# Atten4Vis/LW-DETR

Hardware: AMD Instinct MI355X
Metric: images/sec (higher is better)
Workload: dtype fp16; 1 GPU; LW-DETR-small inference forward + PostProcess, 640x640, batch 32/GPU, fp16, random-init weights (synthetic COCO-shaped input); global_batch=32, per_gpu_batch=32, parallelism=dp1, collective=none, launch_chains=2

## Files before the change

lw-detr_amd/csrc/mlp.hip:

```cpp
#include "common.h"
#include "vit_block_few384.h"
#include <atomic>
#include <cstdlib>
#include <type_traits>

#ifndef MLP_WAVES_PER_SIMD
#define MLP_WAVES_PER_SIMD 2
#endif

#define TSTAMP(i) do {} while (0)

namespace {

#ifndef MLP_NW
#define MLP_NW 8
#endif
#ifndef MLP_TT384
#define MLP_TT384 1
#endif
constexpr int NW = MLP_NW, NTHR = NW * 64;

__device__ __forceinline__ void dma16(const void* sbase, unsigned voff, const void* lds_wave_base) {
    const unsigned m0v = __builtin_amdgcn_readfirstlane(
        (unsigned)(uintptr_t)(__attribute__((address_space(3))) const void*)lds_wave_base);
    asm volatile("s_mov_b32 m0, %0\n\ts_nop 0\n\tglobal_load_lds_dwordx4 %1, %2" :: "s"(m0v), "v"(voff), "s"(sbase) : "memory");
}
__device__ __forceinline__ const void* uniform_ptr(const void* p) {
    const uintptr_t v = (uintptr_t)p;
    const unsigned lo = __builtin_amdgcn_readfirstlane((unsigned)v), hi = __builtin_amdgcn_readfirstlane((unsigned)(v >> 32));
    return (const void*)(((uintptr_t)hi << 32) | lo);
}
__device__ __forceinline__ void dma_sync() {
    asm volatile("s_waitcnt vmcnt(0)" ::: "memory");
    __syncthreads();
}

struct MlpParams {
    void* x; long ldx;
    const void* w1; const float* b1;
    const void* w2p; const float* b2;
    const float* gamma2;
    void* out2; long ld2;
    float* stats_out;
    long M; float eps, eps_next;
    int ntiles;
    const void* att; long ldatt; const void* wp; const float* bp; const float* gamma1;
    const void* wqkv; const float* bqkv; void* q; void* k; void* vt; float qscale; int heads, hd, Tp;
    float* partial; int chunks_per_split;
    int wfrag;
};

constexpr int MP_COUNT = 44;
std::atomic<long> g_mlp_path[MP_COUNT];
const char* const kMlpPathNames[MP_COUNT] = {
    "mlp_f16_c192_proj0_qkv0", "mlp_f16_c192_proj1_qkv0", "mlp_f16_c192_proj1_qkv1", "mlp_f16_c384_proj0_qkv0", "mlp_f16_c384_proj1_qkv0",
    "mlp_f16_c384_proj1_qkv1", "mlp_bf16_c192_proj0_qkv0", "mlp_bf16_c192_proj1_qkv0", "mlp_bf16_c192_proj1_qkv1", "mlp_bf16_c384_proj0_qkv0",
    "mlp_bf16_c384_proj1_qkv0", "mlp_bf16_c384_proj1_qkv1", "mlp_f32_c192_proj0_qkv0", "mlp_f32_c192_proj1_qkv0", "mlp_f32_c192_proj1_qkv1",
    "mlp_f32_c384_proj0_qkv0", "mlp_f32_c384_proj1_qkv0", "mlp_f32_c384_proj1_qkv1", "mlp_small_f16_tt1_qkv0_frag0", "mlp_small_f16_tt1_qkv0_frag1",
    "mlp_small_f16_tt1_qkv1_frag0", "mlp_small_f16_tt1_qkv1_frag1", "mlp_small_f16_tt2_qkv0_frag0", "mlp_small_f16_tt2_qkv0_frag1", "mlp_small_f16_tt2_qkv1_frag0",
    "mlp_small_f16_tt2_qkv1_frag1", "mlp_small_bf16_tt1_qkv0_frag0", "mlp_small_bf16_tt1_qkv0_frag1", "mlp_small_bf16_tt1_qkv1_frag0",
    "mlp_small_bf16_tt1_qkv1_frag1", "mlp_small_bf16_tt2_qkv0_frag0", "mlp_small_bf16_tt2_qkv0_frag1", "mlp_small_bf16_tt2_qkv1_frag0",
    "mlp_small_bf16_tt2_qkv1_frag1", "mlp_small_f32_tt1_qkv0_frag1", "mlp_small_f32_tt1_qkv1_frag1", "vit_few384_f16_qkv0", "vit_few384_f16_qkv1",
    "vit_few384_bf16_qkv0", "vit_few384_bf16_qkv1", "ffn_f16_c256", "ffn_f16_c384", "ffn_bf16_c256", "ffn_bf16_c384"};
template <typename T> constexpr int mp_dt() { return std::is_same<T, f16>::value ? 0 : (std::is_same<T, bf16>::value ? 1 : 2); }
template <typename T, int C, bool PROJ, bool QKV> constexpr int mp_mlp() {
    static_assert((C == 192 || C == 384) && (PROJ || !QKV), "a form the record has no name for");
    return (mp_dt<T>() * 2 + (C == 384 ? 1 : 0)) * 3 + (PROJ ? (QKV ? 2 : 1) : 0);
}
template <typename T, bool QKV, int TT, bool FRAG> constexpr int mp_small() {
    static_assert(TT == 1 || TT == 2, "");
    static_assert(mp_dt<T>() < 2 || (TT == 1 && FRAG), "the f32 few-token kernel is built with TT = 1 on fragment-major weights only");
    return mp_dt<T>() == 2 ? 34 + (QKV ? 1 : 0) : 18 + ((mp_dt<T>() * 2 + (TT - 1)) * 2 + (QKV ? 1 : 0)) * 2 + (FRAG ? 1 : 0);
}
inline int mp_few384(int dtype, bool qkv) { return 36 + (dtype == DT_F16 ? 0 : 2) + (qkv ? 1 : 0); }
template <typename T, int C> constexpr int mp_ffn() {
    static_assert(mp_dt<T>() < 2 && (C == 256 || C == 384), "");
    return 40 + mp_dt<T>() * 2 + (C == 384 ? 1 : 0);
}
inline int mlp_path_done(int path, int rc) {
    if (rc == LWDETR_OK && path >= 0 && path < MP_COUNT) g_mlp_path[path].fetch_add(1, std::memory_order_relaxed);
    return rc;
}

template <typename T, int C, int TT, bool PROJ, bool QKV, bool FFN = false>
__global__ __launch_bounds__(NTHR, MLP_WAVES_PER_SIMD) void mlp_kernel(const MlpParams p) {
    static_assert(!FFN || (!PROJ && !QKV), "FFN mode has no projection / chained QKV");
    typedef typename Vec<T>::v8 V8;
    typedef typename Vec<T>::v4 V4;
    constexpr int KC = C / 32;
    constexpr int NT = C / 16;
    constexpr int HID = 4 * C, NCH = HID / 32;
    constexpr int EPC = 16 / (int)sizeof(T);
    constexpr int W1_LD = C + 2 * EPC;
// ... 104 lines not shown
        V8 af[TT][KC];
#pragma unroll
        for (int t = 0; t < TT; ++t) {
            long m = m_wave + t * 16 + l15; m = m < p.M ? m : p.M - 1;
            const T* ar = ATT + m * p.ldatt + g * 8;
#pragma unroll
            for (int kc = 0; kc < KC; ++kc) af[t][kc] = *(const V8*)(ar + kc * 32);
        }
        dma_sync();
#pragma unroll
        for (int pc = 0; pc < KC; ++pc) {
            const int buf = pc & 1;
            if (pc + 1 < KC) stage_rows32(WP + (long)(pc + 1) * 32 * C, buf ^ 1);
            else stage_w(0, buf ^ 1);
            const T* wps = smem + buf * TILE_STRIDE;
            f32x4 accp[2][TT];
#pragma unroll
            for (int h = 0; h < 2; ++h)
#pragma unroll
                for (int t = 0; t < TT; ++t) accp[h][t] = f32x4{0.f, 0.f, 0.f, 0.f};
#pragma unroll
            for (int kc = 0; kc < KC; ++kc)
#pragma unroll
                for (int h = 0; h < 2; ++h) {
                    const V8 a = *(const V8*)(wps + (h * 16 + l15) * W1_LD + kc * 32 + g * 8);
#pragma unroll
                    for (int t = 0; t < TT; ++t) accp[h][t] = Mma<T>::k32(a, af[t][kc], accp[h][t]);
                }
#pragma unroll
            for (int h = 0; h < 2; ++h) {
                const int c0 = pc * 32 + h * 16 + g * 4;
                const f32x4 bb = *(const f32x4*)(bps + c0), gg = *(const f32x4*)(bps + C + c0);
#pragma unroll
                for (int t = 0; t < TT; ++t) {
                    const long m = m_wave + t * 16 + l15;
                    const long mr = m < p.M ? m : p.M - 1;
                    V4 x1;
                    if (X1LDS) {
                        T* xs = x1s + (t * 16 + l15) * X1_LD + c0;
                        x1 = cvt4<T>(up4<T>(*(const V4*)xs) + gg * (accp[h][t] + bb));
                        if (wave < X1_TILES) *(V4*)xs = x1;
                    } else {
                        x1 = cvt4<T>(up4<T>(*(const V4*)(X + mr * p.ldx + c0)) + gg * (accp[h][t] + bb));
                        if (m < p.M) *(V4*)(X + m * p.ldx + c0) = x1;
                    }
#pragma unroll
                    for (int e = 0; e < 4; ++e) xf[t][pc][h * 4 + e] = x1[e];
                }
            }
            dma_sync();
        }
    }
    TSTAMP(1);
#pragma unroll
    for (int t = 0; t < (FFN ? 0 : TT); ++t) {
        float s = 0.f;
#pragma unroll
        for (int kc = 0; kc < KC; ++kc)
#pragma unroll
            for (int e = 0; e < 8; ++e) s += to_f32<T>(xf[t][kc][e]);
        s += __shfl_xor(s, 16); s += __shfl_xor(s, 32);
        const float mean = s * (1.f / C);
        float v = 0.f;
#pragma unroll
        for (int kc = 0; kc < KC; ++kc)
#pragma unroll
            for (int e = 0; e < 8; ++e) { const float dl = to_f32<T>(xf[t][kc][e]) - mean; v += dl * dl; }
        v += __shfl_xor(v, 16); v += __shfl_xor(v, 32);
        const float rstd = 1.f / sqrtf(v * (1.f / C) + p.eps);
#pragma unroll
        for (int kc = 0; kc < KC; ++kc)
#pragma unroll
            for (int e = 0; e < 8; ++e) xf[t][kc][e] = from_f32<T>((to_f32<T>(xf[t][kc][e]) - mean) * rstd);
    }

    f32x4 acc2[NT][TT];
#pragma unroll
    for (int n = 0; n < NT; ++n)
#pragma unroll
        for (int t = 0; t < TT; ++t) acc2[n][t] = f32x4{0.f, 0.f, 0.f, 0.f};

    if (!PROJ) dma_sync();
    TSTAMP(2);
    for (int hc = hc0; hc < hc1; ++hc) {
        const int buf = (hc - hc0) & 1;
        if (hc + 1 < hc1) stage_w(hc + 1, buf ^ 1);
        const T* w1s = smem + buf * TILE_STRIDE;
        const T* w2s = w1s + W1_TILE_PAD;
        const f32x4 bia0 = *(const f32x4*)(b1s + (hc - hc0) * 32 + g * 4), bia1 = *(const f32x4*)(b1s + (hc - hc0) * 32 + 16 + g * 4);
        constexpr int RD = 3, NF1 = 2 * KC, NF = NF1 + NT;
        auto frag = [&](int i) -> V8 {
            if (i < NF1) return *(const V8*)(w1s + ((i & 1) * 16 + l15) * W1_LD + (i >> 1) * 32 + g * 8);
            return *(const V8*)(w2s + ((i - NF1) * 16 + l15) * W2_LD + g * 8);
        };
        V8 fr[RD];
#pragma unroll
        for (int i = 0; i < RD; ++i) fr[i] = frag(i);
        f32x4 acc1[2][TT];
#pragma unroll
        for (int t = 0; t < TT; ++t) { acc1[0][t] = bia0; acc1[1][t] = bia1; }
#pragma unroll
        for (int i = 0; i < NF1; ++i) {
            const V8 a = fr[i % RD];
            fr[i % RD] = frag(i + RD);
#pragma unroll
            for (int t = 0; t < TT; ++t) acc1[i & 1][t] = Mma<T>::k32(a, xf[t][i >> 1], acc1[i & 1][t]);
            __builtin_amdgcn_sched_barrier(0);
        }
        V8 hf[TT];
#pragma unroll
        for (int t = 0; t < TT; ++t)
#pragma unroll
            for (int e = 0; e < 4; ++e) {
                hf[t][e] = from_f32<T>(FFN ? fmaxf(acc1[0][t][e], 0.f) : gelu_for<T>(acc1[0][t][e]));
                hf[t][4 + e] = from_f32<T>(FFN ? fmaxf(acc1[1][t][e], 0.f) : gelu_for<T>(acc1[1][t][e]));
            }
        __builtin_amdgcn_sched_barrier(0);
#pragma unroll
        for (int n = 0; n < NT; ++n) {
            const int i = NF1 + n;
            const V8 a = fr[i % RD];
            if (i + RD < NF) fr[i % RD] = frag(i + RD);
#pragma unroll
            for (int t = 0; t < TT; ++t) acc2[n][t] = Mma<T>::k32(a, hf[t], acc2[n][t]);
            __builtin_amdgcn_sched_barrier(0);
        }
        dma_sync();
    }

    TSTAMP(3);
    if (FFN) {
        float* __restrict__ part = p.partial + (long)blockIdx.y * p.M * C;
#pragma unroll
        for (int t = 0; t < TT; ++t) {
            const long m = m_wave + t * 16 + l15;
            if (m < p.M) {
#pragma unroll
                for (int n = 0; n < NT; ++n) *(f32x4*)(part + m * C + n * 16 + g * 4) = acc2[n][t];
            }
        }
        return;
    }
    T* __restrict__ O2 = (T*)p.out2;
    V8 xq[QKV ? TT : 1][QKV ? KC : 1];
#pragma unroll
    for (int t = 0; t < TT; ++t) {
        const long m = m_wave + t * 16 + l15;
        const bool ok = m < p.M;
        const long mr = ok ? m : p.M - 1;
#pragma unroll
        for (int n = 0; n < NT; ++n) {
            const int c0 = n * 16 + g * 4;
            const f32x4 b2 = X1LDS ? *(const f32x4*)(b2s + c0) : *(const f32x4*)(p.b2 + c0);
            const f32x4 g2 = X1LDS ? *(const f32x4*)(b2s + C + c0) : *(const f32x4*)(p.gamma2 + c0);
            const f32x4 xr = up4<T>(X1LDS ? *(const V4*)(x1s + (t * 16 + l15) * X1_LD + c0) : *(const V4*)(X + mr * p.ldx + c0));
            acc2[n][t] = up4<T>(cvt4<T>(xr + g2 * (acc2[n][t] + b2)));
        }
        if (ok) {
#pragma unroll
            for (int n = 0; n < NT; ++n) {
                const V4 o = cvt4<T>(acc2[n][t]);
                *(V4*)(X + m * p.ldx + n * 16 + g * 4) = o;
                if (O2) *(V4*)(O2 + m * p.ld2 + n * 16 + g * 4) = o;
            }
        }
        if (p.stats_out || QKV) {
            float s = 0.f;
#pragma unroll
            for (int n = 0; n < NT; ++n) s += acc2[n][t][0] + acc2[n][t][1] + acc2[n][t][2] + acc2[n][t][3];
            s += __shfl_xor(s, 16); s += __shfl_xor(s, 32);
            const float mean = s * (1.f / C);
            float v = 0.f;
#pragma unroll
            for (int n = 0; n < NT; ++n)
#pragma unroll
                for (int e = 0; e < 4; ++e) { const float dl = acc2[n][t][e] - mean; v += dl * dl; }
            v += __shfl_xor(v, 16); v += __shfl_xor(v, 32);
            const float rstd = 1.f / sqrtf(v * (1.f / C) + p.eps_next);
            if (p.stats_out && ok && g == 0) { p.stats_out[2 * m] = mean; p.stats_out[2 * m + 1] = rstd; }
            if (QKV) {
#pragma unroll
                for (int kc = 0; kc < KC; ++kc)
#pragma unroll
                    for (int e = 0; e < 4; ++e) {
                        xq[t][kc][e] = from_f32<T>((acc2[2 * kc][t][e] - mean) * rstd);
                        xq[t][kc][4 + e] = from_f32<T>((acc2[2 * kc + 1][t][e] - mean) * rstd);
                    }
            }
        }
    }
    TSTAMP(4);
    if (QKV) {
        constexpr int XLD = C + 2 * EPC;
        constexpr int NTQ = 3 * C / 16, NJ = (NTQ + NW - 1) / NW;
        const T* __restrict__ WQ = (const T*)p.wqkv;
        T* __restrict__ Qo = (T*)p.q; T* __restrict__ Ko = (T*)p.k; T* __restrict__ Vo = (T*)p.vt;
        if (X1LDS) __syncthreads();
        constexpr int FRAG_REGS = KC * (int)sizeof(V8) / 4;
        constexpr int JP = (120 / FRAG_REGS) < 1 ? 1 : ((120 / FRAG_REGS) > NJ ? NJ : (120 / FRAG_REGS));
#pragma unroll
        for (int t = 0; t < TT; ++t)
#pragma unroll
            for (int kc = 0; kc < KC; ++kc)
                *(V8*)(smem + ((wave * TT + t) * 16 + l15) * XLD + kc * 32 + g * 8) = xq[t][kc];
        __syncthreads();
        TSTAMP(5);
        const long m_blk = (long)tile0 * (16 * TT);
        const int ntt = my_tiles * TT;
#pragma unroll 1
        for (int j0 = 0; j0 < NJ; j0 += JP) {
            V8 wq[JP][KC];
#pragma unroll
            for (int j = 0; j < JP; ++j) {
                const int nt = wave + NW * (j0 + j);
                const T* wr = WQ + (long)((nt < NTQ ? nt : NTQ - 1) * 16 + l15) * C + g * 8;
#pragma unroll
                for (int kc = 0; kc < KC; ++kc) wq[j][kc] = *(const V8*)(wr + kc * 32);
            }
            long coff[JP]; float4 cbias[JP]; int csg[JP];
#pragma unroll
            for (int j = 0; j < JP; ++j) {
                const int nt = wave + NW * (j0 + j);
                const int ntc = nt < NTQ ? nt : NTQ - 1;
                const int sg = ntc / (C / 16), nl0 = (ntc - sg * (C / 16)) * 16;
                csg[j] = nt < NTQ ? sg : -1;
                if (sg < 2) {
                    const int nl = nl0 + g * 4, hh = nl / p.hd, dd = nl - hh * p.hd;
                    coff[j] = (long)hh * p.Tp * p.hd + dd;
                    const f32x4 bb = *(const f32x4*)(bqs + sg * C + nl);
                    cbias[j] = make_float4(bb[0], bb[1], bb[2], bb[3]);
                } else {
                    const int nl = nl0 + l15, hh = nl / p.hd, dd = nl - hh * p.hd;
                    coff[j] = ((long)hh * p.hd + dd) * p.Tp;
                    const float bb = bqs[2 * C + nl];
                    cbias[j] = make_float4(bb, bb, bb, bb);
                }
            }
#pragma unroll 1
            for (int tt = 0; tt < ntt; ++tt) {
                V8 xr[KC];
#pragma unroll
                for (int kc = 0; kc < KC; ++kc) xr[kc] = *(const V8*)(smem + (tt * 16 + l15) * XLD + kc * 32 + g * 8);
                const int mq = (int)m_blk + tt * 16 + l15, mv = (int)m_blk + tt * 16 + g * 4;
                const int bq_ = mq / p.Tp, bv_ = mv / p.Tp;
                const long roff_qk = ((long)bq_ * p.heads * p.Tp + (mq - bq_ * p.Tp)) * p.hd;
                const long roff_v = (long)bv_ * p.heads * p.hd * p.Tp + (mv - bv_ * p.Tp);
                const bool okq = mq < p.M, okv = mv < p.M;
#pragma unroll
                for (int j = 0; j < JP; ++j) {
                    if (csg[j] < 0) continue;
                    f32x4 acc = {cbias[j].x, cbias[j].y, cbias[j].z, cbias[j].w};
                    if (csg[j] < 2) {
#pragma unroll
                        for (int kc = 0; kc < KC; ++kc) acc = Mma<T>::k32(wq[j][kc], xr[kc], acc);
                        if (okq) {
                            T* dst = csg[j] == 0 ? Qo : Ko;
                            *(V4*)(dst + roff_qk + coff[j]) = cvt4<T>(acc * (csg[j] == 0 ? p.qscale : 1.f));
                        }
                    } else {
#pragma unroll
                        for (int kc = 0; kc < KC; ++kc) acc = Mma<T>::k32(xr[kc], wq[j][kc], acc);
                        if (okv) *(V4*)(Vo + roff_v + coff[j]) = cvt4<T>(acc);
                    }
                }
            }
        }
    }
    TSTAMP(6);
}

template <typename T, bool QKV, int TT, bool FRAG = false>
__global__ __launch_bounds__(NTHR, 1) void mlp_small_kernel(const MlpParams p) {
    constexpr int C = 192, KC = C / 32, NT = C / 16, HID = 4 * C, X1_LD = C + 8;
    auto frag = [&](const T* w, int rt, int kc, int l15_, int g_) { return FRAG ? w + ((long)(rt * KC + kc) * 16 + l15_) * 32 + g_ * 8 : w + (long)(rt * 16 + l15_) * C + kc * 32 + g_ * 8; };
    typedef typename Vec<T>::v8 V8;
    typedef typename Vec<T>::v4 V4;
    static_assert(sizeof(T) == 2, "");
    extern __shared__ __attribute__((aligned(16))) char smem_raw[];
    T* x1s = (T*)smem_raw;
    float* part = (float*)(x1s + 16 * TT * X1_LD);
    float* b1s = part + NW * 6 * TT * 256;
    float* bps = b1s + HID; float* bqs = bps + 2 * C; float* b2s = bqs + 3 * C;
    const int tid = threadIdx.x, lane = tid & 63, wave = __builtin_amdgcn_readfirstlane(tid >> 6);
    const int l15 = lane & 15, g = lane >> 4;
    const long m0 = (long)blockIdx.x * (16 * TT);
    T* __restrict__ X = (T*)p.x;
    const T* __restrict__ W1 = (const T*)p.w1;
    const T* __restrict__ W2 = (const T*)p.w2p;
    for (int i = tid; i < HID; i += NTHR) b1s[i] = p.b1[i];
    for (int i = tid; i < C; i += NTHR) { bps[i] = p.bp[i]; bps[C + i] = p.gamma1[i]; b2s[i] = p.b2[i]; b2s[C + i] = p.gamma2[i]; }
    if (QKV) for (int i = tid; i < 3 * C; i += NTHR) bqs[i] = p.bqkv[i];
    long mrow[TT]; bool mok[TT];
#pragma unroll
    for (int t = 0; t < TT; ++t) { const long m = m0 + t * 16 + l15; mok[t] = m < p.M; mrow[t] = mok[t] ? m : p.M - 1; }
    __syncthreads();

    if (wave < KC) {
        const int pc = wave;
        const T* __restrict__ ATT = (const T*)p.att;
        const T* __restrict__ WP = (const T*)p.wp;
        V8 af[TT][KC], wa[2][KC];
        V4 xr[2][TT];
#pragma unroll
        for (int t = 0; t < TT; ++t)
#pragma unroll
            for (int kc = 0; kc < KC; ++kc) af[t][kc] = *(const V8*)(ATT + mrow[t] * p.ldatt + kc * 32 + g * 8);
#pragma unroll
        for (int h = 0; h < 2; ++h) {
#pragma unroll
            for (int kc = 0; kc < KC; ++kc) wa[h][kc] = *(const V8*)frag(WP, pc * 2 + h, kc, l15, g);
#pragma unroll
            for (int t = 0; t < TT; ++t) xr[h][t] = *(const V4*)(X + mrow[t] * p.ldx + pc * 32 + h * 16 + g * 4);
        }
#pragma unroll
        for (int h = 0; h < 2; ++h) {
            const int c0 = pc * 32 + h * 16 + g * 4;
            const f32x4 bb = *(const f32x4*)(bps + c0), gg = *(const f32x4*)(bps + C + c0);
#pragma unroll
            for (int t = 0; t < TT; ++t) {
                f32x4 a = {0.f, 0.f, 0.f, 0.f};
#pragma unroll
                for (int kc = 0; kc < KC; ++kc) a = Mma<T>::k32(wa[h][kc], af[t][kc], a);
                *(V4*)(x1s + (t * 16 + l15) * X1_LD + c0) = cvt4<T>(up4<T>(xr[h][t]) + gg * (a + bb));
            }
        }
    }
    __syncthreads();

    V8 xf[TT][KC];
#pragma unroll
    for (int t = 0; t < TT; ++t)
#pragma unroll
        for (int kc = 0; kc < KC; ++kc)
#pragma unroll
            for (int h = 0; h < 2; ++h) {
                const V4 v = *(const V4*)(x1s + (t * 16 + l15) * X1_LD + kc * 32 + h * 16 + g * 4);
#pragma unroll
                for (int e = 0; e < 4; ++e) xf[t][kc][h * 4 + e] = v[e];
            }
#pragma unroll
    for (int t = 0; t < TT; ++t) {
        float sm = 0.f;
#pragma unroll
        for (int kc = 0; kc < KC; ++kc)
#pragma unroll
            for (int e = 0; e < 8; ++e) sm += to_f32<T>(xf[t][kc][e]);
        sm += __shfl_xor(sm, 16); sm += __shfl_xor(sm, 32);
        const float mean = sm * (1.f / C);
        float v = 0.f;
#pragma unroll
        for (int kc = 0; kc < KC; ++kc)
// ... 369 lines not shown
            const int mq = (int)m0 + l15, bq_ = mq / p.Tp;
            if (mq < p.M) {
                float* dst = (sg == 0 ? Qo : Ko) + ((long)bq_ * p.heads * p.Tp + (mq - bq_ * p.Tp)) * p.hd + (long)hh * p.Tp * p.hd + dd;
                *(f32x4*)dst = acc * (sg == 0 ? p.qscale : 1.f);
            }
        } else {
            const int nl = nl0 + l15, hh = nl / p.hd, dd = nl - hh * p.hd;
            const float bb = bqs[2 * C + nl];
            f32x4 acc = {bb, bb, bb, bb};
#pragma unroll
            for (int kc = 0; kc < KC; ++kc) acc = Mma<float>::k32(xq[kc], wq[it & 1][kc], acc);
            const int mv = (int)m0 + g * 4, bv_ = mv / p.Tp;
            if (mv < p.M)
                *(f32x4*)(Vo + (long)bv_ * p.heads * p.hd * p.Tp + (mv - bv_ * p.Tp) + ((long)hh * p.hd + dd) * p.Tp) = acc;
        }
    }
}
template <> __global__ __launch_bounds__(NTHR, 1) void mlp_small_kernel<float, true, 1, true>(const MlpParams p) { mlp_small_f32<true>(p); }
template <> __global__ __launch_bounds__(NTHR, 1) void mlp_small_kernel<float, false, 1, true>(const MlpParams p) { mlp_small_f32<false>(p); }

constexpr size_t MLP_LDS_MAX = 160 * 1024;
constexpr long MLP_SMALL_TT1_MAX_ROWS = 3200;
template <typename T, bool QKV, int TT, bool FRAG = false>
int launch_mlp_small_tt(const MlpParams& p, hipStream_t st) {
    constexpr int C = 192;
    constexpr size_t lds = 16 * TT * (C + 8) * sizeof(T) + (size_t)NW * 6 * TT * 256 * sizeof(float) + 11 * C * sizeof(float);
    static bool attr_done[16] = {};
    int dev = 0;
    if (hipGetDevice(&dev) != hipSuccess || dev < 0 || dev >= 16) return LWDETR_ERR_LAUNCH;
    if (!attr_done[dev]) {
        if (hipFuncSetAttribute((const void*)mlp_small_kernel<T, QKV, TT, FRAG>, hipFuncAttributeMaxDynamicSharedMemorySize, (int)lds) != hipSuccess)
            return LWDETR_ERR_LAUNCH;
        attr_done[dev] = true;
    }
    const long blocks = (p.M + 16 * TT - 1) / (16 * TT);
    ProfScope ps(KID_MLP, (16.0 + 2.0 + (QKV ? 6.0 : 0.0)) * p.M * C * C, (double)p.M * C * sizeof(T) * 3 + (QKV ? 3.0 : 0.0) * p.M * C * sizeof(T), st);
    hipLaunchKernelGGL((mlp_small_kernel<T, QKV, TT, FRAG>), dim3((unsigned)blocks), dim3(NTHR), lds, st, p);
    return mlp_path_done(mp_small<T, QKV, TT, FRAG>(), lwdetr_check_launch());
}
template <typename T, bool QKV>
int launch_mlp_small(const MlpParams& p, hipStream_t st) {
    const int tt = (int)lwdetr_knob(KNOB_MLP_SMALL_TT, p.M <= MLP_SMALL_TT1_MAX_ROWS ? 1 : 2);
    if (p.wfrag) return tt == 1 ? launch_mlp_small_tt<T, QKV, 1, true>(p, st) : launch_mlp_small_tt<T, QKV, 2, true>(p, st);
    return tt == 1 ? launch_mlp_small_tt<T, QKV, 1>(p, st) : launch_mlp_small_tt<T, QKV, 2>(p, st);
}

template <typename T, int C, int TT, bool PROJ, bool QKV>
int launch_mlp_p(const MlpParams& p, hipStream_t st) {
    constexpr int EPC = 16 / (int)sizeof(T);
    constexpr int PIECE = 64 * EPC;
    constexpr int W1P = (32 * (C + 2 * EPC) + PIECE - 1) / PIECE * PIECE, W2P = (C * (32 + 2 * EPC) + PIECE - 1) / PIECE * PIECE;
    constexpr size_t tiles_b = 2 * (size_t)(W1P + W2P) * sizeof(T);
    constexpr size_t xchg_b = QKV ? (size_t)NW * 16 * TT * (C + 2 * EPC) * sizeof(T) : 0;
    constexpr bool X1LDS = PROJ && sizeof(T) == 2 && C == 192;
    constexpr int X1_TILES = 7;
    constexpr size_t x1_b = X1LDS ? (size_t)X1_TILES * 16 * TT * (C + 8) * sizeof(T) : 0;
    constexpr size_t lds = (tiles_b + x1_b > xchg_b ? tiles_b + x1_b : xchg_b) + (9 + (X1LDS ? 2 : 0)) * C * sizeof(float);
    if constexpr (lds > MLP_LDS_MAX) return LWDETR_ERR_UNSUPPORTED;
    static int ncu_dev[16] = {};
    int dev = 0;
    if (hipGetDevice(&dev) != hipSuccess || dev < 0 || dev >= 16) return LWDETR_ERR_LAUNCH;
    if (!ncu_dev[dev]) {
        hipDeviceProp_t prop;
        if (hipFuncSetAttribute((const void*)mlp_kernel<T, C, TT, PROJ, QKV>, hipFuncAttributeMaxDynamicSharedMemorySize, (int)lds) != hipSuccess ||
            hipGetDeviceProperties(&prop, dev) != hipSuccess)
            return LWDETR_ERR_LAUNCH;
        ncu_dev[dev] = prop.multiProcessorCount > 0 ? prop.multiProcessorCount : 256;
    }
    const int ncu = ncu_dev[dev];
    MlpParams q = p;
    q.ntiles = (int)((p.M + 16 * TT - 1) / (16 * TT));
    long blocks = q.ntiles < ncu ? q.ntiles : ncu;
    constexpr int TPW = X1LDS ? X1_TILES : NW;
    if ((long)q.ntiles > blocks * TPW) blocks = (q.ntiles + TPW - 1) / TPW;
    ProfScope ps(KID_MLP, (16.0 + (PROJ ? 2.0 : 0.0) + (QKV ? 6.0 : 0.0)) * p.M * C * C,
                 (double)p.M * C * sizeof(T) * (PROJ ? 3 : 2) + (QKV ? 3.0 : 0.0) * p.M * C * sizeof(T), st);
    hipLaunchKernelGGL((mlp_kernel<T, C, TT, PROJ, QKV>), dim3((unsigned)blocks), dim3(NTHR), lds, st, q);
    return mlp_path_done(mp_mlp<T, C, PROJ, QKV>(), lwdetr_check_launch());
}

constexpr int FFN_MAX_SPLITS = 16;
template <typename T, int C, int TT>
int launch_ffn(const MlpParams& p0, int hid, hipStream_t st, int* splits_out) {
    constexpr int EPC = 16 / (int)sizeof(T);
    constexpr int PIECE = 64 * EPC;
    constexpr int W1P = (32 * (C + 2 * EPC) + PIECE - 1) / PIECE * PIECE, W2P = (C * (32 + 2 * EPC) + PIECE - 1) / PIECE * PIECE;
    constexpr size_t lds = 2 * (size_t)(W1P + W2P) * sizeof(T) + 9 * C * sizeof(float);
    static int ncu_dev[16] = {};
    int dev = 0;
    if (hipGetDevice(&dev) != hipSuccess || dev < 0 || dev >= 16) return LWDETR_ERR_LAUNCH;
    if (!ncu_dev[dev]) {
        hipDeviceProp_t prop;
        if (hipFuncSetAttribute((const void*)mlp_kernel<T, C, TT, false, false, true>, hipFuncAttributeMaxDynamicSharedMemorySize, (int)lds) != hipSuccess ||
            hipGetDeviceProperties(&prop, dev) != hipSuccess)
            return LWDETR_ERR_LAUNCH;
        ncu_dev[dev] = prop.multiProcessorCount > 0 ? prop.multiProcessorCount : 256;
    }
    const int ncu = ncu_dev[dev];
    MlpParams q = p0;
    q.ntiles = (int)((p0.M + 16 * TT - 1) / (16 * TT));
    int blocks = (q.ntiles + NW - 1) / NW;
    const int nch = hid / 32;
    int S = 1;
    while ((long)(nch / S) * 32 > 4 * C && nch % (S * 2) == 0) S *= 2;
    if ((long)(nch / S) * 32 > 4 * C) return LWDETR_ERR_UNSUPPORTED;
    const int s_max = (int)lwdetr_knob(KNOB_FFN_SPLITS, FFN_MAX_SPLITS);
    while (S * 2 * blocks <= ncu && nch % (S * 2) == 0 && nch / (S * 2) >= 2 && S * 2 <= s_max) S *= 2;
    if (ncu / S > blocks) blocks = ncu / S < q.ntiles ? ncu / S : q.ntiles;
    q.chunks_per_split = nch / S;
    if (splits_out) { *splits_out = S; return LWDETR_OK; }
    ProfScope ps(KID_MLP, 4.0 * p0.M * C * hid, (double)p0.M * C * (sizeof(T) + 4.0 * S) + 2.0 * C * hid * sizeof(T), st);
    hipLaunchKernelGGL((mlp_kernel<T, C, TT, false, false, true>), dim3((unsigned)blocks, (unsigned)S), dim3(NTHR), lds, st, q);
    return mlp_path_done(mp_ffn<T, C>(), lwdetr_check_launch());
}

constexpr long MLP_SMALL_MAX_ROWS = 12800;

template <typename T, int C, int TT>
int launch_mlp(const MlpParams& p, hipStream_t st) {
    if constexpr (sizeof(T) == 2 && C == 192) {
        const bool small_ok = p.att && (lwdetr_knob_is_set(KNOB_MLP_SMALL) ? lwdetr_knob(KNOB_MLP_SMALL, 0) == 1 : p.M < MLP_SMALL_MAX_ROWS);
        if (small_ok) return p.wqkv ? launch_mlp_small<T, true>(p, st) : launch_mlp_small<T, false>(p, st);
    }
    if (p.att && p.wqkv) return launch_mlp_p<T, C, TT, true, true>(p, st);
    if (p.att) return launch_mlp_p<T, C, TT, true, false>(p, st);
    if (p.wqkv) return LWDETR_ERR_UNSUPPORTED;
    return launch_mlp_p<T, C, TT, false, false>(p, st);
}

template <typename T, int TT16, int TT32>
int dispatch_c(const MlpParams& p, int C, hipStream_t st) {
    switch (C) {
        case 192: return launch_mlp<T, 192, TT16>(p, st);
        case 384: return launch_mlp<T, 384, TT32>(p, st);
        default: return LWDETR_ERR_UNSUPPORTED;
    }
}

}

extern "C" int lwdetr_mlp_fused(void* x, long ldx, const void* w1_folded, const float* b1_folded, const void* w2_chunked,
                                const float* b2, const float* gamma2, void* out2, long ld2, float* stats_out, long M,
                                int C, float eps, float eps_next, const void* att, long ldatt, const void* wp,
                                const float* bp, const float* gamma1, const void* wqkv_next, const float* bqkv_next,
                                void* q_out, void* k_out, void* vt_out, float qscale, int heads, int hd, int Tp,
                                int dtype, void* hip_stream) {
    if (!x || !w1_folded || !b1_folded || !w2_chunked || !b2 || !gamma2 || M < 0) return LWDETR_ERR_BAD_ARG;
    if (M == 0) return LWDETR_OK;
    if (ldx % 8 != 0 || (out2 && ld2 % 8 != 0)) return LWDETR_ERR_BAD_ARG;
    if (att && (!wp || !bp || !gamma1 || ldatt % 8 != 0)) return LWDETR_ERR_BAD_ARG;
    MlpParams p;
    p.wfrag = 0;
    p.att = att; p.ldatt = ldatt; p.wp = wp; p.bp = bp; p.gamma1 = gamma1;
    p.wqkv = wqkv_next; p.bqkv = bqkv_next; p.q = q_out; p.k = k_out; p.vt = vt_out; p.qscale = qscale;
    p.heads = heads; p.hd = hd; p.Tp = Tp;
    if (wqkv_next && (!bqkv_next || !q_out || !k_out || !vt_out || heads <= 0 || hd % 4 != 0 || heads * hd != C || Tp % 4 != 0 ||
                      M % 4 != 0))
        return LWDETR_ERR_BAD_ARG;
    p.x = x; p.ldx = ldx; p.w1 = w1_folded; p.b1 = b1_folded; p.w2p = w2_chunked; p.b2 = b2; p.gamma2 = gamma2;
    p.out2 = out2; p.ld2 = ld2; p.stats_out = stats_out; p.M = M; p.eps = eps; p.eps_next = eps_next;
    hipStream_t st = (hipStream_t)hip_stream;
    switch (dtype) {
        case DT_F16: return dispatch_c<f16, 2, MLP_TT384>(p, C, st);
        case DT_BF16: return dispatch_c<bf16, 2, MLP_TT384>(p, C, st);
        case DT_F32: return dispatch_c<float, 1, 1>(p, C, st);
        default: return LWDETR_ERR_UNSUPPORTED;
    }
}

extern "C" int lwdetr_vit_block_few(void* x, long ldx, const void* w1_frag, const float* b1_folded, const void* w2_chunked, const float* b2,
                                    const float* gamma2, void* out2, long ld2, float* stats_out, long M, int C, float eps, float eps_next,
                                    const void* att, long ldatt, const void* wp_frag, const float* bp, const float* gamma1,
                                    const void* wqkv_frag_next, const float* bqkv_next, void* q_out, void* k_out, void* vt_out, float qscale,
                                    int heads, int hd, int Tp, int dtype, void* hip_stream) {
    if (!x || !w1_frag || !b1_folded || !w2_chunked || !b2 || !gamma2 || !att || !wp_frag || !bp || !gamma1 || M < 0) return LWDETR_ERR_BAD_ARG;
    if (M == 0) return LWDETR_OK;
    if ((C != 192 && C != 384) || (dtype != DT_F32 && dtype != DT_F16 && dtype != DT_BF16) || M >= MLP_SMALL_MAX_ROWS) return LWDETR_ERR_UNSUPPORTED;
    if (C == 384 && dtype == DT_F32) return LWDETR_ERR_UNSUPPORTED;
    if (dtype == DT_F32) {
        auto mis = [](const void* q) { return ((size_t)q & 15) != 0; };
        if (ldx % 4 != 0 || (out2 && ld2 % 4 != 0) || ldatt % 4 != 0 || mis(x) || mis(att) || mis(out2) || mis(w1_frag) || mis(wp_frag) || mis(wqkv_frag_next) ||
            mis(w2_chunked) || mis(b1_folded) || mis(b2) || mis(bp) || mis(gamma1) || mis(gamma2) || mis(bqkv_next) || mis(q_out) || mis(k_out) || mis(vt_out))
            return LWDETR_ERR_UNSUPPORTED;
    } else if (ldx % 8 != 0 || (out2 && ld2 % 8 != 0) || ldatt % 8 != 0) return LWDETR_ERR_BAD_ARG;
    if (wqkv_frag_next && (!bqkv_next || !q_out || !k_out || !vt_out || heads <= 0 || hd % 4 != 0 || heads * hd != C || Tp % 4 != 0 || M % 4 != 0))
        return LWDETR_ERR_BAD_ARG;
    MlpParams p;
    p.wfrag = 1;
    p.att = att; p.ldatt = ldatt; p.wp = wp_frag; p.bp = bp; p.gamma1 = gamma1;
    p.wqkv = wqkv_frag_next; p.bqkv = bqkv_next; p.q = q_out; p.k = k_out; p.vt = vt_out; p.qscale = qscale;
    p.heads = heads; p.hd = hd; p.Tp = Tp;
    p.x = x; p.ldx = ldx; p.w1 = w1_frag; p.b1 = b1_folded; p.w2p = w2_chunked; p.b2 = b2; p.gamma2 = gamma2;
    p.out2 = out2; p.ld2 = ld2; p.stats_out = stats_out; p.M = M; p.eps = eps; p.eps_next = eps_next;
    p.partial = nullptr; p.chunks_per_split = 0; p.ntiles = 0;
    hipStream_t st = (hipStream_t)hip_stream;
// ... 52 lines not shown
```

Before: 13850 images/sec.

## Add dedicated split-K FFN partial kernel with 5-slot swizzled weight pipeline

Replaces the generic mlp_kernel FFN path with a specialised ffn_partial_kernel. It stages W1/W2 tiles through a 5-slot ring of XOR-swizzled LDS buffers using global_load_lds DMA, with explicit waitcnt/barrier boundaries, so several chunks are in flight at once. Row tiles are spread evenly across blocks and waves, with per-wave unit counts of 0/1/2. The aim is to hide weight-load latency and bank conflicts, at the cost of more LDS use and greater complexity. Optional timing instrumentation is compiled in only under a macro.

```diff
diff --git a/lw-detr_amd/csrc/mlp.hip b/lw-detr_amd/csrc/mlp.hip
--- a/lw-detr_amd/csrc/mlp.hip
+++ b/lw-detr_amd/csrc/mlp.hip
@@ -8,7 +8,18 @@
 #define MLP_WAVES_PER_SIMD 2
 #endif
 
+#ifdef LWDETR_FFN_TIMING
+__device__ unsigned long long g_ffn_timing[2][8][8];
+#define FFN_TNOW() __builtin_amdgcn_s_memrealtime()
+#define FFN_TREC(i, v) do { if (lane == 0 && ((blockIdx.x == 0 && blockIdx.y == 0) || (blockIdx.x == gridDim.x - 1 && blockIdx.y == gridDim.y - 1))) \
+        g_ffn_timing[blockIdx.x != 0 || blockIdx.y != 0][wave & 7][i] = (v); } while (0)
+#define TSTAMP(i) do { if (FFN && (i) <= 4) FFN_TREC(i, FFN_TNOW()); } while (0)
+extern "C" int lwdetr_debug_ffn_timing(unsigned long long* out) {
+    return hipMemcpyFromSymbol(out, HIP_SYMBOL(g_ffn_timing), sizeof(g_ffn_timing)) == hipSuccess ? 0 : 1;
+}
+#else
 #define TSTAMP(i) do {} while (0)
+#endif
 
 namespace {
 
@@ -279,6 +290,9 @@
 
     if (!PROJ) dma_sync();
     TSTAMP(2);
+#ifdef LWDETR_FFN_TIMING
+    unsigned long long t_sync = 0;
+#endif
     for (int hc = hc0; hc < hc1; ++hc) {
         const int buf = (hc - hc0) & 1;
         if (hc + 1 < hc1) stage_w(hc + 1, buf ^ 1);
@@ -322,10 +336,19 @@
             for (int t = 0; t < TT; ++t) acc2[n][t] = Mma<T>::k32(a, hf[t], acc2[n][t]);
             __builtin_amdgcn_sched_barrier(0);
         }
+#ifdef LWDETR_FFN_TIMING
+        const unsigned long long t_s0 = FFN_TNOW();
+#endif
         dma_sync();
+#ifdef LWDETR_FFN_TIMING
+        t_sync += FFN_TNOW() - t_s0;
+#endif
     }
 
     TSTAMP(3);
+#ifdef LWDETR_FFN_TIMING
+    if (FFN) { FFN_TREC(5, t_sync); FFN_TREC(6, 0ull); }
+#endif
     if (FFN) {
         float* __restrict__ part = p.partial + (long)blockIdx.y * p.M * C;
 #pragma unroll
@@ -336,6 +359,7 @@
                 for (int n = 0; n < NT; ++n) *(f32x4*)(part + m * C + n * 16 + g * 4) = acc2[n][t];
             }
         }
+        TSTAMP(4);
         return;
     }
     T* __restrict__ O2 = (T*)p.out2;
@@ -464,6 +488,190 @@
         }
     }
     TSTAMP(6);
+}
+
+constexpr int FFN_NSLOT = 5;
+#ifdef LWDETR_FFN_TIMING
+#define FFN_BOUNDARY(N) do { const unsigned long long t_a = FFN_TNOW(); asm volatile("s_waitcnt vmcnt(%0) lgkmcnt(0)" :: "n"(N) : "memory"); \
+        const unsigned long long t_b = FFN_TNOW(); asm volatile("s_barrier" ::: "memory"); t_wait += t_b - t_a; t_bar += FFN_TNOW() - t_b; } while (0)
+#else
+#define FFN_BOUNDARY(N) asm volatile("s_waitcnt vmcnt(%0) lgkmcnt(0)\n\ts_barrier" :: "n"(N) : "memory")
+#endif
+template <typename T, int C, int NU>
+__device__ __forceinline__ void ffn_partial_wave(const MlpParams& p, const int wave, const long m_wave) {
+    typedef typename Vec<T>::v8 V8;
+    constexpr int TT = NU > 0 ? NU : 1;
+    constexpr bool active = NU > 0;
+    constexpr int KC = C / 32, NT = C / 16;
+    constexpr int TILE = 32 * C;
+    constexpr int PW = TILE / (512 * NW);
+    constexpr int ROW1 = C / 8;
+    static_assert(sizeof(T) == 2 && C % 128 == 0 && TILE % (512 * NW) == 0 && (PW == 2 || PW == 3 || PW == 4 || PW == 6), "");
+    extern __shared__ __attribute__((aligned(16))) char smem_raw[];
+    T* smem = (T*)smem_raw;
+    float* b1s = (float*)(smem + FFN_NSLOT * TILE);
+
+    const int tid = threadIdx.x, lane = tid & 63;
+    const int l15 = lane & 15, g = lane >> 4;
+#ifdef LWDETR_FFN_TIMING
+    unsigned long long t_wait = 0, t_bar = 0;
+    FFN_TREC(0, FFN_TNOW());
+#endif
+    const int nch = p.chunks_per_split, hc0 = (int)blockIdx.y * nch;
+    const T* __restrict__ X = (const T*)p.x;
+    const T* __restrict__ W1 = (const T*)p.w1 + (long)hc0 * TILE;
+    const T* __restrict__ W2 = (const T*)p.w2p + (long)hc0 * TILE;
+
+    unsigned off1[PW], off2[PW];
+#pragma unroll
+    for (int k = 0; k < PW; ++k) {
+        const int ps = (wave + NW * k) * 64 + lane;
+        const int r1 = ps / ROW1, c1 = (ps - r1 * ROW1) ^ ((r1 & 7) << 1);
+        off1[k] = (unsigned)((r1 * C + c1 * 8) * sizeof(T));
+        const int r2 = ps >> 2, c2 = (ps & 3) ^ ((r2 >> 2) & 2);
+        off2[k] = (unsigned)((r2 * 32 + c2 * 8) * sizeof(T));
+    }
+    auto stage = [&](int j, int slot) {
+        const T* src = ((j & 1) ? W2 : W1) + (long)(j >> 1) * TILE;
+        T* dst = smem + slot * TILE;
+#pragma unroll
+        for (int k = 0; k < PW; ++k) dma16(src, (j & 1) ? off2[k] : off1[k], dst + (wave + NW * k) * 512);
+    };
+    const int npiece = 2 * nch;
+    V8 xf[TT][KC] = {};
+    if (active) {
+#pragma unroll
+        for (int t = 0; t < TT; ++t) {
+            long m = m_wave + t * 16 + l15; m = m < p.M ? m : p.M - 1;
+            const T* xr = X + m * p.ldx + g * 8;
+#pragma unroll
+            for (int kc = 0; kc < KC; ++kc) xf[t][kc] = *(const V8*)(xr + kc * 32);
+        }
+    }
+    constexpr int BPT = (4 * C + NTHR - 1) / NTHR;
+    float bv[BPT];
+#pragma unroll
+    for (int k = 0; k < BPT; ++k) { const int i = tid + k * NTHR; bv[k] = i < nch * 32 ? p.b1[hc0 * 32 + i] : 0.f; }
+    stage(0, 0);
+    if (npiece > 1) stage(1, 1);
+#pragma unroll
+    for (int k = 0; k < BPT; ++k) { const int i = tid + k * NTHR; if (i < nch * 32) b1s[i] = bv[k]; }
+#ifdef LWDETR_FFN_TIMING
+    FFN_TREC(1, FFN_TNOW());
+#endif
+    asm volatile("s_waitcnt vmcnt(0) lgkmcnt(0)\n\ts_barrier" ::: "memory");
+#pragma unroll
+    for (int t = 0; t < TT; ++t)
+#pragma unroll
+        for (int kc = 0; kc < KC; ++kc) asm volatile("" : "+v"(xf[t][kc]));
+#ifdef LWDETR_FFN_TIMING
+    FFN_TREC(2, FFN_TNOW());
+#endif
+
+    f32x4 acc2[NT][TT];
+#pragma unroll
+    for (int n = 0; n < NT; ++n)
+#pragma unroll
+        for (int t = 0; t < TT; ++t) acc2[n][t] = f32x4{0.f, 0.f, 0.f, 0.f};
+
+    int a1[4];
+#pragma unroll
+    for (int q = 0; q < 4; ++q) a1[q] = l15 * C + (((q * 4 + g) ^ ((l15 & 7) << 1)) * 8);
+    const int a2 = l15 * 32 + ((g ^ ((l15 >> 2) & 2)) * 8);
+
+    int s1 = 0;
+    for (int c = 0; c < nch; ++c) {
+        if (c == 0) {
+#pragma unroll
+            for (int j = 2; j < FFN_NSLOT; ++j) if (j < npiece) stage(j, j);
+        } else {
+            if (c + 1 < nch) FFN_BOUNDARY(PW);
+            else FFN_BOUNDARY(0);
+            const int sa = s1 >= 2 ? s1 - 2 : s1 + FFN_NSLOT - 2, sb = s1 >= 1 ? s1 - 1 : s1 + FFN_NSLOT - 1;
+            if (2 * c + 3 < npiece) stage(2 * c + 3, sa);
+            if (2 * c + 4 < npiece) stage(2 * c + 4, sb);
+        }
+        const int s2 = s1 + 1 < FFN_NSLOT ? s1 + 1 : 0;
+        if (active) {
+            const T* w1s = smem + s1 * TILE;
+            const T* w2s = smem + s2 * TILE;
+            const f32x4 bia0 = *(const f32x4*)(b1s + c * 32 + g * 4), bia1 = *(const f32x4*)(b1s + c * 32 + 16 + g * 4);
+            constexpr int RD = 3, NF1 = 2 * KC, NF = NF1 + NT;
+            auto frag = [&](int i) -> V8 {
+                if (i < NF1) return *(const V8*)(w1s + a1[(i >> 1) & 3] + (i & 1) * 16 * C + (i >> 3) * 128);
+                return *(const V8*)(w2s + a2 + (i - NF1) * 512);
+            };
+            V8 fr[RD];
+#pragma unroll
+            for (int i = 0; i < RD; ++i) fr[i] = frag(i);
+            f32x4 acc1[2][TT];
+#pragma unroll
+            for (int t = 0; t < TT; ++t) { acc1[0][t] = bia0; acc1[1][t] = bia1; }
+#pragma unroll
+            for (int i = 0; i < NF1; ++i) {
+                const V8 a = fr[i % RD];
+                fr[i % RD] = frag(i + RD);
+#pragma unroll
+                for (int t = 0; t < TT; ++t) acc1[i & 1][t] = Mma<T>::k32(a, xf[t][i >> 1], acc1[i & 1][t]);
+                __builtin_amdgcn_sched_barrier(0);
+            }
+            V8 hf[TT];
+#pragma unroll
+            for (int t = 0; t < TT; ++t)
+#pragma unroll
+                for (int e = 0; e < 4; ++e) {
+                    hf[t][e] = from_f32<T>(fmaxf(acc1[0][t][e], 0.f));
+                    hf[t][4 + e] = from_f32<T>(fmaxf(acc1[1][t][e], 0.f));
+                }
+            __builtin_amdgcn_sched_barrier(0);
+#pragma unroll
+            for (int n = 0; n < NT; ++n) {
+                const int i = NF1 + n;
+                const V8 a = fr[i % RD];
+                if (i + RD < NF) fr[i % RD] = frag(i + RD);
+#pragma unroll
+                for (int t = 0; t < TT; ++t) acc2[n][t] = Mma<T>::k32(a, hf[t], acc2[n][t]);
+                __builtin_amdgcn_sched_barrier(0);
+            }
+        }
+        s1 = s1 + 2 < FFN_NSLOT ? s1 + 2 : s1 + 2 - FFN_NSLOT;
+    }
+#ifdef LWDETR_FFN_TIMING
+    FFN_TREC(3, FFN_TNOW());
+#endif
+    if (active) {
+        float* __restrict__ part = p.partial + (long)blockIdx.y * p.M * C;
+#pragma unroll
+        for (int t = 0; t < TT; ++t) {
+            const long m = m_wave + t * 16 + l15;
+            if (m < p.M) {
+#pragma unroll
+                for (int n = 0; n < NT; ++n) *(f32x4*)(part + m * C + n * 16 + g * 4) = acc2[n][t];
+            }
+        }
+    }
+#ifdef LWDETR_FFN_TIMING
+    FFN_TREC(4, FFN_TNOW()); FFN_TREC(5, t_wait); FFN_TREC(6, t_bar); FFN_TREC(7, (unsigned long long)NU);
+#endif
+}
+
+template <typename T, int C, int TT>
+__global__ __launch_bounds__(NTHR, MLP_WAVES_PER_SIMD) void ffn_partial_kernel(const MlpParams p) {
+    const int wave = __builtin_amdgcn_readfirstlane((int)threadIdx.x >> 6);
+    const int tb = p.ntiles / (int)gridDim.x, tr = p.ntiles % (int)gridDim.x;
+    const int my_tiles = tb + ((int)blockIdx.x < tr ? 1 : 0);
+    const int tile0 = (int)blockIdx.x * tb + ((int)blockIdx.x < tr ? (int)blockIdx.x : tr);
+    const long row0 = (long)tile0 * (16 * TT);
+    const long rows = p.M - row0 < (long)my_tiles * (16 * TT) ? p.M - row0 : (long)my_tiles * (16 * TT);
+    const int units = (int)((rows + 15) / 16);
+    const int ub = units / NW, ur = units % NW;
+    const int mine = ub + (wave < ur ? 1 : 0);
+    const long m_wave = row0 + 16 * (long)(wave * ub + (wave < ur ? wave : ur));
+    if constexpr (TT == 2) {
+        if (mine == 2) return ffn_partial_wave<T, C, 2>(p, wave, m_wave);
+    }
+    if (mine >= 1) return ffn_partial_wave<T, C, 1>(p, wave, m_wave);
+    ffn_partial_wave<T, C, 0>(p, wave, m_wave);
 }
 
 template <typename T, bool QKV, int TT, bool FRAG = false>
@@ -999,16 +1207,22 @@
 constexpr int FFN_MAX_SPLITS = 16;
 template <typename T, int C, int TT>
 int launch_ffn(const MlpParams& p0, int hid, hipStream_t st, int* splits_out) {
+#ifdef LWDETR_FFN_PARENT
     constexpr int EPC = 16 / (int)sizeof(T);
     constexpr int PIECE = 64 * EPC;
     constexpr int W1P = (32 * (C + 2 * EPC) + PIECE - 1) / PIECE * PIECE, W2P = (C * (32 + 2 * EPC) + PIECE - 1) / PIECE * PIECE;
     constexpr size_t lds = 2 * (size_t)(W1P + W2P) * sizeof(T) + 9 * C * sizeof(float);
+    const auto kernel = mlp_kernel<T, C, TT, false, false, true>;
+#else
+    constexpr size_t lds = (size_t)FFN_NSLOT * 32 * C * sizeof(T) + 4 * C * sizeof(float);
+    const auto kernel = ffn_partial_kernel<T, C, TT>;
+#endif
     static int ncu_dev[16] = {};
     int dev = 0;
     if (hipGetDevice(&dev) != hipSuccess || dev < 0 || dev >= 16) return LWDETR_ERR_LAUNCH;
     if (!ncu_dev[dev]) {
         hipDeviceProp_t prop;
-        if (hipFuncSetAttribute((const void*)mlp_kernel<T, C, TT, false, false, true>, hipFuncAttributeMaxDynamicSharedMemorySize, (int)lds) != hipSuccess ||
+        if (hipFuncSetAttribute((const void*)kernel, hipFuncAttributeMaxDynamicSharedMemorySize, (int)lds) != hipSuccess ||
             hipGetDeviceProperties(&prop, dev) != hipSuccess)
             return LWDETR_ERR_LAUNCH;
         ncu_dev[dev] = prop.multiProcessorCount > 0 ? prop.multiProcessorCount : 256;
@@ -1027,7 +1241,7 @@
     q.chunks_per_split = nch / S;
     if (splits_out) { *splits_out = S; return LWDETR_OK; }
     ProfScope ps(KID_MLP, 4.0 * p0.M * C * hid, (double)p0.M * C * (sizeof(T) + 4.0 * S) + 2.0 * C * hid * sizeof(T), st);
-    hipLaunchKernelGGL((mlp_kernel<T, C, TT, false, false, true>), dim3((unsigned)blocks, (unsigned)S), dim3(NTHR), lds, st, q);
+    hipLaunchKernelGGL(kernel, dim3((unsigned)blocks, (unsigned)S), dim3(NTHR), lds, st, q);
     return mlp_path_done(mp_ffn<T, C>(), lwdetr_check_launch());
 }
 
```

New measurement: 13910 images/sec (median of 6 runs). About the same (+0.4%).
